# XiSHEN0220/RANSAC-Flow

Measured on AMD Instinct MI355X. Metric: aligned image-pairs/sec @480×640, 1/2/4/8 MI355X; max-abs flow Δ vs ref, higher is better.
Workload: dtype f32

## Files before the change

ransac-flow_amd/csrc/conv1x1s.hip:

```cpp
#include "common.h"
#include "conv_epilogue.h"
#include "group.h"

namespace {

typedef __bf16 bf16x8 __attribute__((ext_vector_type(8)));
typedef __bf16 bf16x2 __attribute__((ext_vector_type(2)));
typedef float f32x2 __attribute__((ext_vector_type(2)));
typedef unsigned u32x4 __attribute__((ext_vector_type(4)));

struct C1SArgs {
    const float* in; const u32x4* wS; const float* scale; const float* shift; const float* res; float* out;
    int Cin, HW, Cout, act, Mpad;
    long long P;
    int tilesM, tilesP;
    int stride, Win, Wo, HWin;
};

__device__ __forceinline__ unsigned pack_bf16(float a, float b) {
    const f32x2 v = {a, b};
    const bf16x2 h = __builtin_convertvector(v, bf16x2);
    unsigned u;
    __builtin_memcpy(&u, &h, 4);
    return u;
}
__device__ __forceinline__ void split_pair(float a, float b, unsigned& hi, unsigned& mid, unsigned& lo) {
    hi = pack_bf16(a, b);
    const float ra = a - __uint_as_float(hi << 16), rb = b - __uint_as_float(hi & 0xffff0000u);
    mid = pack_bf16(ra, rb);
    lo = pack_bf16(ra - __uint_as_float(mid << 16), rb - __uint_as_float(mid & 0xffff0000u));
}
__device__ __forceinline__ bf16x8 as_frag(const u32x4& w) {
    bf16x8 f;
    __builtin_memcpy(&f, &w, 16);
    return f;
}

template <int TM>
__device__ __forceinline__ void conv1x1_split_body(const C1SArgs& a, const unsigned bx) {
    constexpr int BM = 64 * TM, BN = 128, KB = 16;
    constexpr int A_WORDS = 3 * 2 * BM;
    constexpr int NA = (A_WORDS + 255) / 256;
    __shared__ u32x4 As[2][3][2][BM];
    __shared__ u32x4 Bs[2][3][2][BN];
    __shared__ float s_scale[BM], s_shift[BM];

    const int t = threadIdx.x, lane = t & 63, wave = t >> 6;
    const int wm = wave >> 1, wn = wave & 1;
    const int lrow = lane >> 5, lcol = lane & 31;
    const size_t HW = (size_t)a.HW, HWin = (size_t)a.HWin;
    const int nwg = a.tilesM * a.tilesP;
    const int nk = a.Cin / KB;

    int m0; long long n0;
    {
        const int v = (int)bx, q = nwg / 8, r = nwg % 8, xcd = v % 8, j = v / 8;
        const int bid = (xcd < r ? xcd * (q + 1) : r * (q + 1) + (xcd - r) * q) + j;
        m0 = (bid % a.tilesM) * BM;
        n0 = (long long)(bid / a.tilesM) * BN;
    }
    constexpr int A_ROWS = 256 / BM;
    const u32x4* wsrc = a.wS + (size_t)(t / BM) * a.Mpad + m0 + t % BM;
    auto a_on = [&](int j) { return (j + 1) * 256 <= A_WORDS || t + 256 * j < A_WORDS; };
    const int bh = t >> 7, bp = t & 127;
    const float* bsrc;
    {
        long long p = n0 + bp;
        if (p >= a.P) p = a.P - 1;
        const long long n = p / a.HW;
        int off = (int)(p - n * a.HW);
        if (a.stride != 1) { const int y = off / a.Wo, x = off - y * a.Wo; off = y * a.stride * a.Win + x * a.stride; }
        bsrc = a.in + ((size_t)n * a.Cin + 8 * bh) * HWin + (size_t)off;
    }
    u32x4 ra[NA];
    float rb[8];
    auto load_stage = [&](int kb) {
#pragma unroll
        for (int j = 0; j < NA; ++j)
            ra[j] = wsrc[((size_t)kb * 6 + (a_on(j) ? A_ROWS * j : 0)) * a.Mpad];
#pragma unroll
        for (int i = 0; i < 8; ++i) rb[i] = bsrc[(size_t)(kb * KB + i) * HWin];
    };
    auto store_stage = [&](int buf) {
#pragma unroll
        for (int j = 0; j < NA; ++j)
            if (a_on(j)) (&As[buf][0][0][0])[t + 256 * j] = ra[j];
        u32x4 hi, mid, lo;
#pragma unroll
        for (int i = 0; i < 4; ++i) {
            unsigned h_, m_, l_;
            split_pair(rb[2 * i], rb[2 * i + 1], h_, m_, l_);
            hi[i] = h_; mid[i] = m_; lo[i] = l_;
        }
        Bs[buf][0][bh][bp] = hi;
        Bs[buf][1][bh][bp] = mid;
        Bs[buf][2][bh][bp] = lo;
    };
    if (t < BM) {
        const int m = m0 + t;
        s_scale[t] = (a.scale && m < a.Cout) ? a.scale[m] : 1.0f;
        s_shift[t] = (a.shift && m < a.Cout) ? a.shift[m] : 0.0f;
    }
    load_stage(0);
    store_stage(0);
    if (nk > 1) load_stage(1);
    __syncthreads();

    f32x16 acc[TM][2], low[TM][2];
#pragma unroll
    for (int i = 0; i < TM; ++i)
#pragma unroll
        for (int j = 0; j < 2; ++j)
#pragma unroll
            for (int r = 0; r < 16; ++r) { acc[i][j][r] = 0.0f; low[i][j][r] = 0.0f; }

    for (int s = 0; s < nk; ++s) {
        const int cur = s & 1;
        bf16x8 af[3][TM], bf[3][2];
#pragma unroll
        for (int pc = 0; pc < 3; ++pc) {
#pragma unroll
            for (int i = 0; i < TM; ++i) af[pc][i] = as_frag(As[cur][pc][lrow][wm * TM * 32 + i * 32 + lcol]);
#pragma unroll
            for (int j = 0; j < 2; ++j) bf[pc][j] = as_frag(Bs[cur][pc][lrow][wn * 64 + j * 32 + lcol]);
        }
        if (s + 1 < nk) store_stage(cur ^ 1);
        if (s + 2 < nk) load_stage(s + 2);
        __builtin_amdgcn_sched_barrier(0);
#pragma unroll
        for (int i = 0; i < TM; ++i)
#pragma unroll
            for (int j = 0; j < 2; ++j) {
                low[i][j] = __builtin_amdgcn_mfma_f32_32x32x16_bf16(af[2][i], bf[0][j], low[i][j], 0, 0, 0);
                low[i][j] = __builtin_amdgcn_mfma_f32_32x32x16_bf16(af[0][i], bf[2][j], low[i][j], 0, 0, 0);
                low[i][j] = __builtin_amdgcn_mfma_f32_32x32x16_bf16(af[1][i], bf[1][j], low[i][j], 0, 0, 0);
            }
#pragma unroll
        for (int i = 0; i < TM; ++i)
#pragma unroll
            for (int j = 0; j < 2; ++j) {
                low[i][j] = __builtin_amdgcn_mfma_f32_32x32x16_bf16(af[1][i], bf[0][j], low[i][j], 0, 0, 0);
                low[i][j] = __builtin_amdgcn_mfma_f32_32x32x16_bf16(af[0][i], bf[1][j], low[i][j], 0, 0, 0);
                acc[i][j] = __builtin_amdgcn_mfma_f32_32x32x16_bf16(af[0][i], bf[0][j], acc[i][j], 0, 0, 0);
            }
        __builtin_amdgcn_sched_barrier(0);
        __syncthreads();
    }
#pragma unroll
    for (int i = 0; i < TM; ++i)
#pragma unroll
        for (int j = 0; j < 2; ++j)
#pragma unroll
            for (int r = 0; r < 16; ++r) acc[i][j][r] += low[i][j][r];

    size_t pix_off[2];
    bool pix_ok[2];
#pragma unroll
    for (int j = 0; j < 2; ++j) {
        long long pp = n0 + wn * 64 + j * 32 + lcol;
        pix_ok[j] = pp < a.P;
        if (!pix_ok[j]) pp = a.P - 1;
        const long long n = pp / a.HW;
        pix_off[j] = (size_t)n * a.Cout * HW + (size_t)(pp - n * a.HW);
    }
    conv_epilogue<TM, 2, false>(acc, s_scale, s_shift, a.res, a.out, a.act, a.Cout, HW, m0, wm, lrow, pix_off, pix_ok, m0 + BM <= a.Cout);
}

template <int TM>
__global__ __launch_bounds__(256, 2) void conv1x1_split_kernel(C1SArgs a) {
    conv1x1_split_body<TM>(a, blockIdx.x);
}

template <int TM>
__global__ __launch_bounds__(256, 2) void conv1x1_split_group_kernel(RfxGroupArgs<C1SArgs> g) {
    const unsigned y = blockIdx.y;
    if (blockIdx.x >= g.gx[y]) return;
    conv1x1_split_body<TM>(g.p[y], blockIdx.x);
}

template <int TM>
static int c1s_group_launch(const void* blob, const unsigned* gx, int n, hipStream_t st) {
    return rfx_group_launch_impl<C1SArgs>(conv1x1_split_group_kernel<TM>, 256, blob, gx, n, st);
}

template <int TM>
int launch_split(C1SArgs& a, hipStream_t st) {
    a.tilesM = (a.Cout + 64 * TM - 1) / (64 * TM);
    a.tilesP = (int)((a.P + 127) / 128);
    const long long nwg = (long long)a.tilesM * a.tilesP;
    if (nwg > 0x7fffffffLL) return RFX_E_LIMIT;
    if (rfx_group_recording()) return rfx_group_record(&c1s_group_launch<TM>, &a, sizeof(a), (unsigned)nwg);
    hipLaunchKernelGGL((conv1x1_split_kernel<TM>), dim3((unsigned)nwg), dim3(256), 0, st, a);
    RFX_LAUNCH_CHECK();
    return RFX_OK;
}

}

static int conv1x1_split_launch(const float* in, const void* wS, const float* scale, const float* shift, const float* residual,
                                float* out, int N, int Cin, int Hin, int Win, int Cout, int stride, int act, void* stream) {
    if (!in || !wS || !out || N <= 0 || Cin <= 0 || Hin <= 0 || Win <= 0 || Cout <= 0) return RFX_E_ARG;
    if (Cin % 16 != 0 || (stride != 1 && stride != 2)) return RFX_E_ARG;
    if (act != RFX_ACT_NONE && act != RFX_ACT_RELU && act != RFX_ACT_SIGMOID) return RFX_E_ARG;
    const int Ho = (Hin - 1) / stride + 1, Wo = (Win - 1) / stride + 1;
    C1SArgs a;
    a.in = in; a.wS = reinterpret_cast<const u32x4*>(wS); a.scale = scale; a.shift = shift; a.res = residual; a.out = out;
    a.Cin = Cin; a.HW = Ho * Wo; a.Cout = Cout; a.act = act; a.Mpad = (Cout + 127) / 128 * 128;
    a.P = (long long)N * a.HW;
    a.stride = stride; a.Win = Win; a.Wo = Wo; a.HWin = Hin * Win;
    return Cout > 64 ? launch_split<2>(a, rfx_stream(stream)) : launch_split<1>(a, rfx_stream(stream));
}

extern "C" int rfx_conv1x1_split_f32(const float* in, const void* wS, const float* scale, const float* shift, const float* residual,
                                     float* out, int N, int Cin, int HW, int Cout, int act, void* stream) {
    return conv1x1_split_launch(in, wS, scale, shift, residual, out, N, Cin, 1, HW, Cout, 1, act, stream);
}

extern "C" int rfx_conv1x1_split_strided_f32(const float* in, const void* wS, const float* scale, const float* shift, const float* residual,
                                             float* out, int N, int Cin, int Hin, int Win, int Cout, int stride, int act, void* stream) {
    return conv1x1_split_launch(in, wS, scale, shift, residual, out, N, Cin, Hin, Win, Cout, stride, act, stream);
}
```

Before: 162.4.

## Stream conv1x1 operands into LDS via direct global-to-LDS DMA with triple-buffered raw stage

Replaces the register-staged global loads with global_load_lds DMA for both the weight tiles and the raw f32 activations. Activations land in a new three-slot LDS ring before being split into bf16 hi/mid/lo. The main loop is rewritten around hand-written ds_read/ds_write asm, explicit vmcnt/lgkmcnt waits and s_barrier, with the last stage peeled off. The aim is to cut VGPR pressure and overlap more global latency with the MFMA work. In exchange it uses more LDS, which could lower occupancy, and the hand-counted waitcnt values are fragile.

New measurement: 165.1, median of 6. 1.7% higher.

```diff
diff --git a/ransac-flow_amd/csrc/conv1x1s.hip b/ransac-flow_amd/csrc/conv1x1s.hip
--- a/ransac-flow_amd/csrc/conv1x1s.hip
+++ b/ransac-flow_amd/csrc/conv1x1s.hip
@@ -1,6 +1,7 @@
 #include "common.h"
 #include "conv_epilogue.h"
 #include "group.h"
+#include <type_traits>
 
 namespace {
 
@@ -36,16 +37,38 @@
     return f;
 }
 
+typedef const __attribute__((address_space(1))) void* gptr_t;
+typedef __attribute__((address_space(3))) void* lptr_t;
+
+template <int OFF>
+__device__ __forceinline__ void lds_rd(u32x4& d, unsigned addr) {
+    asm volatile("ds_read_b128 %0, %1 offset:%2" : "=v"(d) : "v"(addr), "n"(OFF));
+}
+template <int OFF0, int OFF1>
+__device__ __forceinline__ void lds_rd2(f32x2& d, unsigned addr) {
+    asm volatile("ds_read2st64_b32 %0, %1 offset0:%2 offset1:%3" : "=v"(d) : "v"(addr), "n"(OFF0), "n"(OFF1));
+}
+__device__ __forceinline__ void lds_wr3(unsigned addr, const u32x4& hi, const u32x4& mid, const u32x4& lo) {
+    asm volatile("ds_write_b128 %0, %1\n\tds_write_b128 %0, %2 offset:4096\n\tds_write_b128 %0, %3 offset:8192\n\ts_nop 1"
+                 :: "v"(addr), "v"(hi), "v"(mid), "v"(lo) : "memory");
+}
+template <typename T>
+__device__ __forceinline__ void tie(T& r) { asm volatile("" : "+v"(r)); }
+
 template <int TM>
 __device__ __forceinline__ void conv1x1_split_body(const C1SArgs& a, const unsigned bx) {
     constexpr int BM = 64 * TM, BN = 128, KB = 16;
     constexpr int A_WORDS = 3 * 2 * BM;
     constexpr int NA = (A_WORDS + 255) / 256;
+    constexpr int B_WORDS = 3 * 2 * BN;
+    constexpr int NR = 3;
+    constexpr int R_BYTES = KB * BN * 4;
     __shared__ u32x4 As[2][3][2][BM];
     __shared__ u32x4 Bs[2][3][2][BN];
+    __shared__ float Rw[NR][KB][BN];
     __shared__ float s_scale[BM], s_shift[BM];
 
-    const int t = threadIdx.x, lane = t & 63, wave = t >> 6;
+    const int t = threadIdx.x, lane = t & 63, wave = __builtin_amdgcn_readfirstlane(t >> 6);
     const int wm = wave >> 1, wn = wave & 1;
     const int lrow = lane >> 5, lcol = lane & 31;
     const size_t HW = (size_t)a.HW, HWin = (size_t)a.HWin;
@@ -61,7 +84,13 @@
     }
     constexpr int A_ROWS = 256 / BM;
     const u32x4* wsrc = a.wS + (size_t)(t / BM) * a.Mpad + m0 + t % BM;
-    auto a_on = [&](int j) { return (j + 1) * 256 <= A_WORDS || t + 256 * j < A_WORDS; };
+    auto dma_w = [&](int kb, int buf) {
+#pragma unroll
+        for (int j = 0; j < NA; ++j)
+            if ((j + 1) * 256 <= A_WORDS || wave < (A_WORDS - 256 * j) / 64)
+                __builtin_amdgcn_global_load_lds((gptr_t)(wsrc + ((size_t)kb * 6 + A_ROWS * j) * a.Mpad),
+                                                 (lptr_t)(&As[buf][0][0][0] + 256 * j + 64 * wave), 16, 0, 0);
+    };
     const int bh = t >> 7, bp = t & 127;
     const float* bsrc;
     {
@@ -72,39 +101,50 @@
         if (a.stride != 1) { const int y = off / a.Wo, x = off - y * a.Wo; off = y * a.stride * a.Win + x * a.stride; }
         bsrc = a.in + ((size_t)n * a.Cin + 8 * bh) * HWin + (size_t)off;
     }
-    u32x4 ra[NA];
-    float rb[8];
-    auto load_stage = [&](int kb) {
-#pragma unroll
-        for (int j = 0; j < NA; ++j)
-            ra[j] = wsrc[((size_t)kb * 6 + (a_on(j) ? A_ROWS * j : 0)) * a.Mpad];
-#pragma unroll
-        for (int i = 0; i < 8; ++i) rb[i] = bsrc[(size_t)(kb * KB + i) * HWin];
-    };
-    auto store_stage = [&](int buf) {
-#pragma unroll
-        for (int j = 0; j < NA; ++j)
-            if (a_on(j)) (&As[buf][0][0][0])[t + 256 * j] = ra[j];
+    auto dma_r = [&](int kb, int slot) {
+        const float* src = bsrc + (size_t)kb * KB * HWin;
+#pragma unroll
+        for (int i = 0; i < 8; ++i)
+            __builtin_amdgcn_global_load_lds((gptr_t)(src + i * HWin), (lptr_t)(&Rw[slot][8 * (wave >> 1) + i][64 * (wave & 1)]), 4, 0, 0);
+    };
+    const unsigned as_lds = (unsigned)(uintptr_t)(lptr_t)&As[0][0][0][0], bs_lds = (unsigned)(uintptr_t)(lptr_t)&Bs[0][0][0][0];
+    const unsigned rw_lds = (unsigned)(uintptr_t)(lptr_t)&Rw[0][0][0] + (unsigned)((8 * bh * BN + bp) * 4);
+    const unsigned bw_lds = bs_lds + (unsigned)((bh * BN + bp) * 16);
+    auto raw_rd = [&](f32x2 (&r)[4], int slot) {
+        const unsigned ad = rw_lds + (unsigned)(slot * R_BYTES);
+        lds_rd2<0, 2>(r[0], ad); lds_rd2<4, 6>(r[1], ad); lds_rd2<8, 10>(r[2], ad); lds_rd2<12, 14>(r[3], ad);
+    };
+    auto split_wr = [&](const f32x2 (&r)[4], int buf) {
         u32x4 hi, mid, lo;
 #pragma unroll
         for (int i = 0; i < 4; ++i) {
             unsigned h_, m_, l_;
-            split_pair(rb[2 * i], rb[2 * i + 1], h_, m_, l_);
+            split_pair(r[i][0], r[i][1], h_, m_, l_);
             hi[i] = h_; mid[i] = m_; lo[i] = l_;
         }
-        Bs[buf][0][bh][bp] = hi;
-        Bs[buf][1][bh][bp] = mid;
-        Bs[buf][2][bh][bp] = lo;
-    };
+        lds_wr3(bw_lds + (unsigned)(buf * B_WORDS * 16), hi, mid, lo);
+    };
+
+    dma_w(0, 0);
+    dma_r(0, 0);
+    if (nk > 1) dma_r(1, 1);
     if (t < BM) {
         const int m = m0 + t;
         s_scale[t] = (a.scale && m < a.Cout) ? a.scale[m] : 1.0f;
         s_shift[t] = (a.shift && m < a.Cout) ? a.shift[m] : 0.0f;
     }
-    load_stage(0);
-    store_stage(0);
-    if (nk > 1) load_stage(1);
-    __syncthreads();
+    asm volatile("s_waitcnt vmcnt(0)" ::: "memory");
+    if (nk > 2) dma_r(2, 2);
+    {
+        f32x2 r[4];
+        raw_rd(r, 0);
+        asm volatile("s_waitcnt lgkmcnt(0)" ::: "memory");
+#pragma unroll
+        for (int i = 0; i < 4; ++i) tie(r[i]);
+        split_wr(r, 0);
+    }
+    asm volatile("s_waitcnt lgkmcnt(0)" ::: "memory");
+    __builtin_amdgcn_s_barrier();
 
     f32x16 acc[TM][2], low[TM][2];
 #pragma unroll
@@ -114,19 +154,49 @@
 #pragma unroll
             for (int r = 0; r < 16; ++r) { acc[i][j][r] = 0.0f; low[i][j][r] = 0.0f; }
 
-    for (int s = 0; s < nk; ++s) {
-        const int cur = s & 1;
+    const unsigned a_base = as_lds + (unsigned)((lrow * BM + wm * TM * 32 + lcol) * 16);
+    const unsigned b_base = bs_lds + (unsigned)((lrow * BN + wn * 64 + lcol) * 16);
+
+    auto stage = [&](int s, auto split_tag) {
+        constexpr bool SPLIT = decltype(split_tag)::value;
+        const unsigned aa = a_base + (unsigned)((s & 1) * A_WORDS * 16), ba = b_base + (unsigned)((s & 1) * B_WORDS * 16);
+        u32x4 fa[3][TM], fb[3][2];
+        f32x2 r[4];
+#pragma unroll
+        for (int i = 0; i < TM; ++i) {
+            if (i == 0) { lds_rd<0>(fa[0][i], aa); lds_rd<2 * BM * 16>(fa[1][i], aa); lds_rd<4 * BM * 16>(fa[2][i], aa); }
+            else { lds_rd<512>(fa[0][i], aa); lds_rd<2 * BM * 16 + 512>(fa[1][i], aa); lds_rd<4 * BM * 16 + 512>(fa[2][i], aa); }
+        }
+        lds_rd<0>(fb[0][0], ba); lds_rd<512>(fb[0][1], ba);
+        lds_rd<2 * BN * 16>(fb[1][0], ba); lds_rd<2 * BN * 16 + 512>(fb[1][1], ba);
+        lds_rd<4 * BN * 16>(fb[2][0], ba); lds_rd<4 * BN * 16 + 512>(fb[2][1], ba);
+        int slot3 = 0;
+        if constexpr (SPLIT) {
+            slot3 = s % NR;
+            raw_rd(r, slot3 == NR - 1 ? 0 : slot3 + 1);
+            dma_w(s + 1, (s + 1) & 1);
+            if (s + NR < nk) dma_r(s + NR, slot3);
+        }
+        __builtin_amdgcn_sched_barrier(0);
+        asm volatile("s_waitcnt lgkmcnt(0)" ::: "memory");
+#pragma unroll
+        for (int pc = 0; pc < 3; ++pc) {
+#pragma unroll
+            for (int i = 0; i < TM; ++i) tie(fa[pc][i]);
+            tie(fb[pc][0]); tie(fb[pc][1]);
+        }
+        if constexpr (SPLIT) {
+#pragma unroll
+            for (int i = 0; i < 4; ++i) tie(r[i]);
+        }
+        __builtin_amdgcn_sched_barrier(0);
         bf16x8 af[3][TM], bf[3][2];
 #pragma unroll
         for (int pc = 0; pc < 3; ++pc) {
 #pragma unroll
-            for (int i = 0; i < TM; ++i) af[pc][i] = as_frag(As[cur][pc][lrow][wm * TM * 32 + i * 32 + lcol]);
-#pragma unroll
-            for (int j = 0; j < 2; ++j) bf[pc][j] = as_frag(Bs[cur][pc][lrow][wn * 64 + j * 32 + lcol]);
-        }
-        if (s + 1 < nk) store_stage(cur ^ 1);
-        if (s + 2 < nk) load_stage(s + 2);
-        __builtin_amdgcn_sched_barrier(0);
+            for (int i = 0; i < TM; ++i) af[pc][i] = as_frag(fa[pc][i]);
+            bf[pc][0] = as_frag(fb[pc][0]); bf[pc][1] = as_frag(fb[pc][1]);
+        }
 #pragma unroll
         for (int i = 0; i < TM; ++i)
 #pragma unroll
@@ -143,9 +213,16 @@
                 low[i][j] = __builtin_amdgcn_mfma_f32_32x32x16_bf16(af[0][i], bf[1][j], low[i][j], 0, 0, 0);
                 acc[i][j] = __builtin_amdgcn_mfma_f32_32x32x16_bf16(af[0][i], bf[0][j], acc[i][j], 0, 0, 0);
             }
-        __builtin_amdgcn_sched_barrier(0);
-        __syncthreads();
-    }
+        if constexpr (SPLIT) {
+            split_wr(r, (s + 1) & 1);
+            __builtin_amdgcn_sched_barrier(0);
+            if (s + NR < nk) asm volatile("s_waitcnt vmcnt(8) lgkmcnt(0)" ::: "memory");
+            else asm volatile("s_waitcnt vmcnt(0) lgkmcnt(0)" ::: "memory");
+            __builtin_amdgcn_s_barrier();
+        }
+    };
+    for (int s = 0; s + 1 < nk; ++s) stage(s, std::true_type{});
+    stage(nk - 1, std::false_type{});
 #pragma unroll
     for (int i = 0; i < TM; ++i)
 #pragma unroll
```
